# liruiw/OMG-Planner

Measured on AMD Instinct MI355X. Metric: CHOMP iterations/sec (batched scenes) + ms/plan, Panda 7-DoF 30-wp, higher is better.
Workload: dtype f32 SDF / f64 kinematics+update; 1 GPU; 100 table-top scenes/GPU x (64-goal goal-set cost + CHOMP step), Panda 9-dof, 30 waypoints; scenes_per_gpu=100, total_scenes=100, goals=64, waypoints=30, sdf_grid=4x64^3 + 128x96x32 per scene, private, goal_selection=MD on device (omgx_goal_update_optimize), pipeline_parts=3, top_k_collision=1000, plan_restart_every_steps=50

## Files before the change

### include/omg_hip.h

```cpp
#ifndef OMG_HIP_H
#define OMG_HIP_H

#include <stdint.h>

#ifdef __cplusplus
extern "C" {
#endif

#define OMGX_OK 0
#define OMGX_ERR_INVALID (-1)
#define OMGX_ERR_LAUNCH (-2)
#define OMGX_ERR_UNSUPPORTED (-3)

#define OMGX_NUM_LINKS 10
#define OMGX_NUM_DOF 9
#define OMGX_MAX_POINTS 16
#define OMGX_MAX_WAYPOINTS 64
#define OMGX_MAX_CONSTRAINTS 8
#define OMGX_INFO_STRIDE 16

#define OMGX_ROBOT_POSE0 0
#define OMGX_ROBOT_TIP2JOINT 160
#define OMGX_ROBOT_CENTER_OFFSET 320
#define OMGX_ROBOT_JOINT_AXIS 480
// ... 188 lines not shown
                         const int32_t* h_dims, float* out, void* stream);

int32_t omgx_goalset_schedule_len(int32_t num_scenes, int32_t num_goals, int32_t slack);
int omgx_goalset_schedule(const uint32_t* work, const int32_t* active, const int32_t* goal_count, int32_t num_scenes,
                          int32_t num_goals, int32_t slack, int32_t* schedule, void* stream);

int omgx_goalset_schedule_parts(const uint32_t* work, const int32_t* active, const int32_t* goal_count, int32_t num_scenes,
                                int32_t num_goals, int32_t parts, int32_t slack, int32_t* schedule, void* stream);

#define OMGX_SCHEDULE_SCENE_MAJOR 0
#define OMGX_SCHEDULE_LONGEST_FIRST 1
#define OMGX_SCHEDULE_LONGEST_FIRST_MAX_ITEMS 8192
int omgx_goalset_schedule_ordered(const uint32_t* work, const int32_t* active, const int32_t* goal_count, int32_t num_scenes,
                                  int32_t num_goals, int32_t parts, int32_t slack, int32_t order, int32_t* schedule, void* stream);

int64_t omgx_region_scratch_bytes(int32_t dx, int32_t dy, int32_t dz);
int omgx_object_set_grid(omgx_object* object, const float* h_lo, const float* h_hi, const int32_t* h_dims, float delta,
                         int64_t grid_offset, void* stream);
int omgx_fit_influence_region(omgx_object* object, const float* grid, const int32_t* h_dims, const float* h_lo, const float* h_hi,
                              float epsilon, float clearance, void* scratch, void* stream);

int64_t omgx_regions_scratch_bytes(int32_t n_fit, int64_t need_bytes);
int omgx_volume_hashes(const omgx_object* objects, int32_t num_objects, const float* pool, uint64_t* hashes, void* stream);
int omgx_fit_influence_regions(omgx_object* objects, int32_t num_objects, const float* pool, const int32_t* fit_list,
                               const int64_t* need_offsets, int32_t n_fit, int64_t max_voxels, const int32_t* copy_src,
                               void* scratch, void* stream);

typedef struct omgx_plan_iter {
    int32_t mode;
    int32_t start_idx;
// ... 143 lines not shown
```

### omg-planner_amd/csrc/omg_kernels.hip

```cpp
#include <hip/hip_runtime.h>
#include <hip/hip_ext.h>

#include <stdint.h>
#include <stdio.h>
#include <stdlib.h>
#include <string.h>

#include <mutex>

#include "omg_device.h"
#include "omg_host.h"

using namespace omg;

struct RawObjects {
    const float* __restrict__ pose_init;
    const float* __restrict__ sdf_grids;
    const float* __restrict__ sdf_limits;
    const float* __restrict__ eps;
    const float* __restrict__ pad;
    const float* __restrict__ clr;
    const float* __restrict__ dis;
};

#define SDF_LOSS_TILE 32

// ... 671 lines not shown
    if (num_scenes <= 0 || num_goals <= 0 || n_remaining <= 0 || n_points <= 0) return 0;
    (void)n_points;
    return gk_workspace_bytes((int64_t)num_scenes * num_goals, n_remaining);
}

#ifndef GS_LAYER_FOLLOW_MIN
#define GS_LAYER_FOLLOW_MIN 16
#endif
struct GsTiling {
    int goal_parts = 1;
    int layer_lg = 5;
    int layer_cb = 0;
    int spread = 0;
    double* wp_pose_out = nullptr;
    void* kin_ws = nullptr;
};

static inline int gs_parts(int n_remaining, int max_parts) {
    const int ntiles = ((n_remaining + 3) / 4) * 5;
    int np = 1;
    while (np * 2 <= max_parts && ntiles / (np * 2) >= 4) np *= 2;
    return np;
}

static std::atomic<int> g_force_goal_waves{0};
extern "C" void omgx_debug_force_goal_waves(int waves) { g_force_goal_waves.store(waves == 4 || waves == 8 ? waves : 0, std::memory_order_relaxed); }
static inline int gs_wide_waves(int PS, int MR, int P) {
    const int force = g_force_goal_waves.load(std::memory_order_relaxed);
    if (force == 4 || GQ_WAVES != 4 || GqLayout(PS, MR, P, 4, false, 8).total > 64 * 1024) return GQ_WAVES;
    return (force == 8 || GqLayout(PS, MR, P, 4, false, GQ_WAVES).total > 53248) ? 8 : GQ_WAVES;
}
static thread_local int g_last_goalset_variant = 0;
extern "C" int omgx_debug_last_goalset_variant(void) { return g_last_goalset_variant; }

template <class K>
static void gs_launch(K* kernel, unsigned grid, unsigned block, uint32_t lds, hipStream_t st, hipEvent_t ev0, hipEvent_t ev1, const ChunkArgs& ca) {
    if (ev0) hipExtLaunchKernelGGL(kernel, dim3(grid), dim3(block), lds, st, ev0, ev1, 0, ca);
    else hipLaunchKernelGGL(kernel, dim3(grid), dim3(block), lds, st, ca);
}

static int launch_goalset(ChunkArgs& ca, int timing_kind, hipStream_t st, const GsTiling& tl = GsTiling()) {
    const int scene_groups = (ca.S + 7) / 8;
    const bool layer = ca.wp_traj != nullptr;
    if (tl.goal_parts < 1 || tl.goal_parts > 8 || tl.layer_lg < 1 || tl.layer_lg > 10 || 10 % tl.layer_lg != 0 || tl.layer_cb < 0) return OMGX_ERR_INVALID;
    ca.spread = tl.spread != 0;
    ca.NG = ca.NCH;
    ca.NP = ca.NG > 0 ? gs_parts(ca.CH, tl.goal_parts) : 1;
    ca.NCH = ca.NG * ca.NP;
// ... 8 lines not shown
            if (want < ca.wp_n) layer_cb_req = want;
        }
        if (layer && layer_cb_req == 0 && !ca.spread && ca.NG > 0 && tl.layer_lg == 5 && (int64_t)ca.S * ca.NCH <= 1024) {
            ca.layer_lg = 10;
            const int want = ca.CH + 1 > GS_LAYER_FOLLOW_MIN ? ca.CH + 1 : GS_LAYER_FOLLOW_MIN;
            if (want < ca.wp_n) layer_cb_req = want;
        }
    }
    ca.layer_cb = layer ? ((layer_cb_req > 0 && layer_cb_req < ca.wp_n) ? layer_cb_req : ca.wp_n) : 1;
    ca.layer_nb = layer ? (ca.wp_n + ca.layer_cb - 1) / ca.layer_cb : 1;
    ca.layer_parts = ca.layer_lg * ca.layer_nb;
    ca.PS = ca.CH + 1; ca.MR = ca.CH; ca.LPW = 10;
    ca.inv_ncfg = 1.0 / (double)(ca.CH + 1);
    if (layer) { if (ca.layer_cb > ca.PS) ca.PS = ca.layer_cb; if (ca.layer_cb > ca.MR) ca.MR = ca.layer_cb; }
    const int64_t per_scene = (int64_t)ca.NCH + (layer ? ca.layer_parts : 0);
    const int64_t grid = ca.spread ? (int64_t)ca.S * per_scene
                                   : (ca.schedule ? (int64_t)ca.sched_len : (int64_t)scene_groups * ca.NCH * 8) +
                                         (layer ? (int64_t)scene_groups * ca.layer_parts * 8 : 0);
    if (grid > 0x7fffffff) return OMGX_ERR_UNSUPPORTED;
    if (grid == 0) return OMGX_OK;
    const bool pre = tl.kin_ws != nullptr && ca.NG > 0 && ca.traj_start != nullptr;
    const int wide = (!ca.spread && !split && !pre && ca.NG > 0) ? gs_wide_waves(ca.PS, ca.MR, ca.P) : GQ_WAVES;
    ca.tbl_n = gq_choose_tbl_n(ca.PS, ca.MR, ca.P, ca.spread, wide);
    const size_t lds = (size_t)GqLayout(ca.PS, ca.MR, ca.P, ca.tbl_n, ca.spread, wide).total;
    if (lds > 64 * 1024) {
        if (!ca.spread) return OMGX_ERR_UNSUPPORTED;
        int rc = allow_big_lds<10>(k_goalset_queue<2, false, true>, "hipFuncSetAttribute(k_goalset_queue)");
        if (rc != OMGX_OK) return rc;
        rc = allow_big_lds<11>(k_goalset_queue<2, false, true, false, true>, "hipFuncSetAttribute(k_goalset_queue)");
        if (rc != OMGX_OK) return rc;
    }
    ca.pre_poses = nullptr; ca.pre_masks = nullptr;
    if (pre) {
        const int64_t goals = (int64_t)ca.S * ca.NG;
// ... 167 lines not shown

struct GoalsetCall {
    const double* robot = nullptr; int32_t n_points = 0;
    const omgx_object* objects = nullptr; const int32_t* scene_begin = nullptr; const float* sdf_pool = nullptr;
    const double* traj_start = nullptr; int64_t traj_start_stride = 0; const double* goals = nullptr;
    int32_t num_scenes = 0, num_goals = 0, n_remaining = 0, soften_fingers = 0;
    double time_interval = 0.0;
    float *goal_cost = nullptr, *collides = nullptr;
    float* potentials = nullptr;
    void* workspace = nullptr;
    const double* layer_traj = nullptr;
    int32_t layer_n = 0, layer_soften = 0;
    float *layer_pot = nullptr, *layer_grad = nullptr, *layer_col = nullptr;
    const int32_t *active = nullptr, *goal_count = nullptr, *schedule = nullptr;
    int32_t schedule_len = 0; uint32_t* work = nullptr;
    void* stream = nullptr;
    GsTiling tiling;
};

static int goalset_cost_impl(const GoalsetCall& a) {
    if (a.num_scenes < 0 || a.num_goals < 0) return OMGX_ERR_INVALID;
    if (a.num_scenes == 0 || (a.num_goals == 0 && !a.layer_traj)) return OMGX_OK;
    if (!a.robot || !a.objects || !a.scene_begin) return OMGX_ERR_INVALID;
    if (a.num_goals > 0 && (!a.traj_start || !a.goals || !a.goal_cost)) return OMGX_ERR_INVALID;
    if (a.n_points < 1 || a.n_points > OMGX_MAX_POINTS || a.n_remaining < 1 || a.n_remaining > OMGX_MAX_WAYPOINTS)
        return OMGX_ERR_UNSUPPORTED;
    if (!(a.time_interval > 0.0) || (a.num_goals > 0 && a.traj_start_stride < 9)) return OMGX_ERR_INVALID;
    hipStream_t st = (hipStream_t)a.stream;
    const int n = a.num_goals > 0 ? a.n_remaining : 0, C = a.num_goals * n;
    if (a.layer_traj) {
// ... 4 lines not shown
    if ((a.active || a.goal_count || a.schedule || a.work) && a.potentials) return OMGX_ERR_UNSUPPORTED;
    ChunkArgs ca{};
    ca.robot = a.robot; ca.objects = a.objects; ca.scene_begin = a.scene_begin; ca.pool = a.sdf_pool;
    ca.S = a.num_scenes; ca.C = C; ca.CH = n; ca.NCH = a.num_goals; ca.P = a.n_points; ca.soften = a.soften_fingers != 0;
    ca.arc = 1; ca.inv_dt = (float)(1.0 / a.time_interval);
    ca.pot = a.potentials; ca.grad = nullptr; ca.col = nullptr; ca.chunk_cost = a.goal_cost; ca.chunk_col = a.collides;
    ca.traj_start = a.traj_start; ca.ts_stride = a.traj_start_stride; ca.goals = a.goals;
    if (a.layer_traj) {
        ca.wp_traj = a.layer_traj; ca.wp_n = a.layer_n; ca.wp_soften = a.layer_soften != 0;
        ca.wp_pot = a.layer_pot; ca.wp_grad = a.layer_grad; ca.wp_col = a.layer_col;
    }
    if (a.schedule && (a.schedule_len < 8 || a.schedule_len % 8 != 0)) return OMGX_ERR_INVALID;
    ca.active = a.active; ca.goal_count = a.goal_count; ca.schedule = a.schedule; ca.sched_len = a.schedule ? a.schedule_len : 0; ca.work = a.work;
    GsTiling tl = a.tiling;
    tl.kin_ws = a.workspace;
    return a.potentials ? launch_chunks(ca, st) : launch_goalset(ca, 0, st, tl);
}

extern "C" int omgx_goalset_cost(const double* robot, int32_t n_points, const omgx_object* objects,
                                 const int32_t* scene_begin, const float* sdf_pool, const double* traj_start,
                                 int64_t traj_start_stride, const double* goals, int32_t num_scenes, int32_t num_goals,
                                 int32_t n_remaining,
                                 double time_interval, int32_t soften_fingers, float* goal_cost, float* potentials,
                                 float* collides, void* workspace, const int32_t* active, const int32_t* goal_count, void* stream) {
    GoalsetCall a;
    a.robot = robot; a.n_points = n_points; a.objects = objects; a.scene_begin = scene_begin; a.sdf_pool = sdf_pool;
    a.traj_start = traj_start; a.traj_start_stride = traj_start_stride; a.goals = goals; a.num_scenes = num_scenes; a.num_goals = num_goals;
    a.n_remaining = n_remaining; a.time_interval = time_interval; a.soften_fingers = soften_fingers;
    a.goal_cost = goal_cost; a.potentials = potentials; a.collides = collides; a.workspace = workspace;
    a.active = active; a.goal_count = goal_count; a.stream = stream;
    return goalset_cost_impl(a);
}

#define SCH_TPB 1024
#define SCH_LDS_ITEMS 14336
struct SchedArgs {
    const uint32_t* work;
    const int32_t* active;
    const int32_t* goal_count;
    int S, G, slack, slots, staged;
    int32_t* sched;
    int np;
    int longest_first;
};

__global__ __launch_bounds__(SCH_TPB) void k_goalset_schedule(SchedArgs a) {
    extern __shared__ unsigned long long sch_lds[];
    const int S = a.S, G = a.G, tid = threadIdx.x;
    unsigned long long* Ws = sch_lds;
    unsigned long long* Wc = Ws + S;
    unsigned long long* offw = Wc + S;
    uint32_t* nval = reinterpret_cast<uint32_t*>(offw + S);
    uint32_t* offp = nval + S;
    uint32_t* srank = offp + S;
    uint32_t* wl = srank + S;
    unsigned char* xs = reinterpret_cast<unsigned char*>(wl + S * G);
    __shared__ unsigned long long tot[2];
    __shared__ uint32_t cnt_all;
    __shared__ uint32_t first[8];
    __shared__ uint32_t first_r[8];
    __shared__ uint32_t cnt_r[8];
    auto item_w = [&](int s, int g) -> uint32_t {
        if (a.staged) return wl[s * G + g];
        if ((a.active && a.active[s] == 0) || (a.goal_count && g / a.np >= a.goal_count[s])) return 0u;
        const uint32_t w = a.work ? a.work[(size_t)s * G + g] : 1u;
        return w ? w : 1u;
    };
    if (tid == 0) { tot[0] = tot[1] = 0ull; cnt_all = 0u; }
    if (tid < 8) { first[tid] = 0xffffffffu; first_r[tid] = 0xffffffffu; cnt_r[tid] = 0u; }
    for (int i = tid; i < a.slots * 8; i += SCH_TPB) a.sched[i] = -1;
    if (a.staged)
        for (int i = tid; i < S * G; i += SCH_TPB) {
            const int s = i / G, g = i - s * G;
            uint32_t w = 0u;
            if (!((a.active && a.active[s] == 0) || (a.goal_count && g / a.np >= a.goal_count[s]))) {
                w = a.work ? a.work[i] : 1u;
                w = w ? w : 1u;
            }
            wl[i] = w;
        }
    __syncthreads();
    for (int s = tid; s < S; s += SCH_TPB) {
        unsigned long long w = 0;
        uint32_t n = 0;
// ... 53 lines not shown
        pos = offp[s] + r;
        const unsigned long long c2 = 2ull * (offw[s] + before) + wclamp(w);
        const unsigned long long xx = (8ull * c2) / (2ull * total_c);
        x = xx > 7 ? 7 : (int)xx;
        const unsigned long long r2 = 2ull * (offr[s] + before_r) + w;
        const unsigned long long xq = (8ull * r2) / (2ull * total_r);
        xr = xq > 7 ? 7 : (int)xq;
    };
    uint32_t kpos[4];
    int kx[4], kxr[4];
    int kept_n = 0;
    for (int i = tid; i < S * G; i += SCH_TPB) {
        const int s = i / G, g = i - s * G;
        const uint32_t w = item_w(s, g);
        uint32_t pos = 0; int x = -1, xr = -1;
        if (w) { place(s, g, w, pos, x, xr); atomicMin(&first[x], pos); atomicMin(&first_r[xr], pos); atomicAdd(&cnt_r[xr], 1u); }
        if (kept_n < 4) { kpos[kept_n] = pos; kx[kept_n] = x; kxr[kept_n] = xr; }
        ++kept_n;
        if (a.longest_first) xs[i] = (unsigned char)(w ? (x | (xr << 4)) : 255);
    }
    __syncthreads();
    bool use_raw = true;
#pragma unroll
    for (int x = 0; x < 8; ++x) use_raw = use_raw && cnt_r[x] <= (uint32_t)a.slots;
    if (a.longest_first) {
        for (int i = tid; i < S * G; i += SCH_TPB) {
            const uint32_t w = wl[i];
            if (!w) continue;
            const int sh = use_raw ? 4 : 0;
            const unsigned char x = (xs[i] >> sh) & 7;
            uint32_t r = 0;
#pragma unroll 4
            for (int j = 0; j < S * G; ++j) r += (wl[j] != 0u && ((xs[j] >> sh) & 7) == x && (wl[j] > w || (wl[j] == w && j < i))) ? 1u : 0u;
            if ((int)r < a.slots) a.sched[(size_t)r * 8 + x] = i;
        }
        return;
    }
    int k = 0;
    for (int i = tid; i < S * G; i += SCH_TPB, ++k) {
// ... 32 lines not shown
    if (parts != 1 && parts != 2 && parts != 4 && parts != 8) return OMGX_ERR_INVALID;
    if (order != OMGX_SCHEDULE_SCENE_MAJOR && order != OMGX_SCHEDULE_LONGEST_FIRST) return OMGX_ERR_INVALID;
    return goalset_schedule_impl(work, active, goal_count, num_scenes, num_goals, parts, slack, schedule, stream, order);
}

static int goalset_schedule_impl(const uint32_t* work, const int32_t* active, const int32_t* goal_count, int32_t num_scenes,
                                 int32_t num_goals_, int32_t parts, int32_t slack, int32_t* schedule, void* stream, int32_t order) {
    if (num_scenes <= 0 || num_goals_ <= 0 || slack < 1 || !schedule) return OMGX_ERR_INVALID;
    const int64_t items64 = (int64_t)num_goals_ * parts;
    if (items64 > 65536) return OMGX_ERR_UNSUPPORTED;
    const int32_t num_goals = (int32_t)items64;
    if ((int64_t)num_scenes * num_goals > 65536 || num_scenes > OMGX_SCHEDULE_MAX_SCENES) return OMGX_ERR_UNSUPPORTED;
    const int items = num_scenes * num_goals;
    const int staged = (items <= SCH_LDS_ITEMS && num_scenes <= 128) ? 1 : 0;
    const int longest_first = (order == OMGX_SCHEDULE_LONGEST_FIRST && staged && items <= OMGX_SCHEDULE_LONGEST_FIRST_MAX_ITEMS) ? 1 : 0;
    SchedArgs a{work, active, goal_count, num_scenes, num_goals, slack, omgx_goalset_schedule_len(num_scenes, num_goals, slack) / 8, staged, schedule, parts, longest_first};
    const size_t lds = (size_t)num_scenes * (3 * sizeof(unsigned long long) + 3 * sizeof(uint32_t)) + (staged ? (size_t)items * sizeof(uint32_t) : 0) +
                       (longest_first ? (size_t)items : 0);
    hipLaunchKernelGGL(k_goalset_schedule, dim3(1), dim3(SCH_TPB), lds, (hipStream_t)stream, a);
    OMGX_CHECK_LAUNCH("k_goalset_schedule");
    return OMGX_OK;
}

extern "C" int omgx_goalset_cost_layer(const double* robot, int32_t n_points, const omgx_object* objects,
                                       const int32_t* scene_begin, const float* sdf_pool, const double* traj_start,
                                       int64_t traj_start_stride, const double* goals, int32_t num_scenes, int32_t num_goals,
                                       int32_t n_remaining, double time_interval, int32_t soften_fingers, float* goal_cost,
                                       float* collides, void* workspace, const double* traj, int32_t n_waypoints,
                                       int32_t layer_soften_fingers, float* layer_potentials, float* layer_grads,
                                       float* layer_collides, const int32_t* active, const int32_t* goal_count,
                                       const int32_t* schedule, int32_t schedule_len, uint32_t* work, void* stream) {
    if (!traj) return OMGX_ERR_INVALID;
    GoalsetCall a;
    a.robot = robot; a.n_points = n_points; a.objects = objects; a.scene_begin = scene_begin; a.sdf_pool = sdf_pool;
    a.traj_start = traj_start; a.traj_start_stride = traj_start_stride; a.goals = goals; a.num_scenes = num_scenes; a.num_goals = num_goals;
    a.n_remaining = n_remaining; a.time_interval = time_interval; a.soften_fingers = soften_fingers;
    a.goal_cost = goal_cost; a.collides = collides; a.workspace = workspace;
    a.layer_traj = traj; a.layer_n = n_waypoints; a.layer_soften = layer_soften_fingers; a.layer_pot = layer_potentials; a.layer_grad = layer_grads; a.layer_col = layer_collides;
    a.active = active; a.goal_count = goal_count; a.schedule = schedule; a.schedule_len = schedule_len; a.work = work; a.stream = stream;
    return goalset_cost_impl(a);
}

extern "C" int omgx_goalset_cost_layer_parts(const double* robot, int32_t n_points, const omgx_object* objects,
                                             const int32_t* scene_begin, const float* sdf_pool, const double* traj_start,
                                             int64_t traj_start_stride, const double* goals, int32_t num_scenes, int32_t num_goals,
                                             int32_t n_remaining, double time_interval, int32_t soften_fingers, float* goal_cost,
                                             float* collides, const double* traj, int32_t n_waypoints,
                                             int32_t layer_soften_fingers, float* layer_potentials, float* layer_grads,
                                             float* layer_collides, const int32_t* active, const int32_t* goal_count,
                                             const int32_t* schedule, int32_t schedule_len, uint32_t* work, int32_t goal_parts,
                                             double* layer_poses, void* workspace, void* stream) {
    if (!traj) return OMGX_ERR_INVALID;
    GoalsetCall a;
    a.robot = robot; a.n_points = n_points; a.objects = objects; a.scene_begin = scene_begin; a.sdf_pool = sdf_pool;
    a.traj_start = traj_start; a.traj_start_stride = traj_start_stride; a.goals = goals; a.num_scenes = num_scenes; a.num_goals = num_goals;
    a.n_remaining = n_remaining; a.time_interval = time_interval; a.soften_fingers = soften_fingers;
    a.goal_cost = goal_cost; a.collides = collides; a.workspace = workspace;
    a.layer_traj = traj; a.layer_n = n_waypoints; a.layer_soften = layer_soften_fingers; a.layer_pot = layer_potentials; a.layer_grad = layer_grads; a.layer_col = layer_collides;
    a.active = active; a.goal_count = goal_count; a.schedule = schedule; a.schedule_len = schedule_len; a.work = work; a.stream = stream;
    a.tiling.goal_parts = goal_parts; a.tiling.wp_pose_out = layer_poses;
    return goalset_cost_impl(a);
}

extern "C" int32_t omgx_goalset_parts(int32_t n_remaining, int32_t goal_parts) {
    if (n_remaining < 1 || goal_parts < 1 || goal_parts > 8) return 0;
    return gs_parts(n_remaining, goal_parts);
}

extern "C" int omgx_goalset_cost_layer_tiled(const double* robot, int32_t n_points, const omgx_object* objects,
                                             const int32_t* scene_begin, const float* sdf_pool, const double* traj_start,
                                             int64_t traj_start_stride, const double* goals, int32_t num_scenes, int32_t num_goals,
                                             int32_t n_remaining, double time_interval, int32_t soften_fingers, float* goal_cost,
                                             float* collides, const double* traj, int32_t n_waypoints, int32_t layer_soften_fingers,
                                             float* layer_potentials, float* layer_grads, float* layer_collides,
                                             const int32_t* active, const int32_t* goal_count, int32_t goal_parts,
                                             int32_t layer_link_groups, int32_t layer_config_block, int32_t spread, double* layer_poses,
// ... 146 lines not shown
```

### omg-planner_amd/engine.py

```python
from __future__ import annotations

import operator

import numpy as np
import torch

from . import _lib, ops
from .config import Config
from .robot import PandaModel
from .scenes import SceneBatch


def shard_range(num_items: int, rank: int, world: int) -> range:
    base, rem = divmod(num_items, world)
    lo = rank * base + min(rank, rem)
    return range(lo, lo + base + (1 if rank < rem else 0))


_SIDE_STREAMS: dict = {}


def _side_stream(device: torch.device, i: int) -> "torch.cuda.Stream":
    key = (device.index if device.index is not None else torch.cuda.current_device(), i)
    st = _SIDE_STREAMS.get(key)
# ... 150 lines not shown
        self.learner_state = ops.learner_state(S, G, dev, goal_counts)
        self.cost_vec = dzeros((S, G), np.float64)
        self.eta = float(np.sqrt(np.log(G + 1) / cfg.optim_steps))
        self._active = torch.from_numpy(np.ones(S, np.int32)).to(dev)
        self._masked = False
        self.step_count = 0
        self.t = 0
        self._scene_flags = dzeros(S, np.int32)
        self.work = dzeros(S * G * (1 if self.latency else self._parts_max), np.int32)
        self.auto_schedule = True
        self.schedule = None
        self._sched_np = 1
        self._gs_launches = 0
        self._measured = False
        self._sched_buf, self._sched_flip, self._sched_age = None, 0, None
        self._uniform_cache = None
        self._ticket_src = [0]
        self._measure_fence = [None]
        with torch.cuda.device(dev):
            self._num_cus = int(_lib.lib().omgx_device_cu_count())
        if self._num_cus <= 0:
            self._num_cus = torch.cuda.get_device_properties(dev).multi_processor_count
        self._parts, self._forked, self._in_plan = None, False, False
        self._hot = None
        self._capturing = False
        self._scratch_state = self._cubic_h = self._cubic_tmp = self._cubic_diff = None

    @property
    def active(self) -> torch.Tensor:
        return self._active
# ... 105 lines not shown
            tot += parts[:, :, j]
        return tot

    def _make_part(self, lo: int, hi: int, stream):
        import copy
        part = object.__new__(ChompEngine)
        part.__dict__.update(self.__dict__)
        part.cfg = copy.copy(self.cfg)
        part.S, part.stream, part._lo = hi - lo, stream, lo
        part._batch_scenes = self.S
        part._parts, part._forked, part.pipeline = None, False, 1
        part._hot = None
        part.scenes = self.scenes.scene_range(lo, hi)
        part.work = torch.zeros(part.S * self.G * (1 if self.latency else self._parts_max), dtype=torch.int32, device=self.device)
        part.schedule, part._gs_launches, part._measured, part._sched_np = None, 0, False, 1
        part._sched_buf, part._sched_flip, part._sched_age = None, 0, None
        part._uniform_cache = None
        if self.goal_count is not None:
            part._goal_counts_host = self._goal_counts_host[lo:hi]
        self._bind_part(part)
        return part

    def _bind_part(self, part):
        lo, hi = part._lo, part._lo + part.S
        for k in self._PART_TENSORS:
            v = getattr(self, k)
            setattr(part, k, None if v is None else v[lo:hi])

    def _refresh_parts(self):
        for part in self._parts or ():
            self._bind_part(part)
# ... 108 lines not shown
                else:
                    self.schedule = self.build_schedule(active=self._mask(), parts=NP, uniform=rebuild == "masked-uniform")
        return (self.schedule if use else None), (self.work[:items] if measure else None)

    def _dispatch_measured(self, NP: int):
        self._measured = True
        with torch.cuda.stream(self.stream):
            self.schedule = self.build_schedule(parts=NP)

    def _goalset_layer(self, prm: _lib.LearnerParams, calls: "ops.IterationCalls", stream: int):
        self._gs_launches += 1
        NP = self._parts_last = max(1, int(prm.cost_parts))
        schedule, work = (None, None) if self.latency else self._dispatch(NP)
        calls.use_layer_poses = self._poses_on
        if work is None:
            calls.goalset_layer(prm.start_idx, self._masked, schedule, None, stream)
            return
        mine = self.stream if self.stream is not None else torch.cuda.current_stream(self.device)
        fence = self._measure_fence
        if fence[0] is not None:
            mine.wait_event(fence[0])
        calls.goalset_layer(prm.start_idx, self._masked, schedule, work, stream)
        fence[0] = mine.record_event()
        self._dispatch_measured(NP)

    def _uniform_schedule(self, parts: int = 1) -> torch.Tensor:
        S, G = self.S, self.G * parts
        if self.goal_count is not None:
            items = np.concatenate([s * G + np.arange(int(c) * parts) for s, c in enumerate(self._goal_counts_host)])
        else:
            items = np.arange(S * G)
        n = len(items)
        pos = np.arange(n)
        x = np.minimum(8 * pos // max(n, 1), 7)
        first = np.searchsorted(x, np.arange(8))
        rank = pos - first[x]
        slots = int(rank.max()) + 1 if n else 1
        sched = np.full(slots * 8, -1, np.int32)
        sched[rank * 8 + x] = items
        return torch.as_tensor(sched, device=self.device)

    def build_schedule(self, active: "torch.Tensor | None" = None, uniform: bool = False, parts: int = 1) -> torch.Tensor:
        self._sched_np = parts
        if self.S * self.G * parts > 65536 or self.S > _lib.SCHEDULE_MAX_SCENES:
            if self._uniform_cache is None:
                self._uniform_cache = {}
            if parts not in self._uniform_cache:
                self._uniform_cache[parts] = self._uniform_schedule(parts)
            return self._uniform_cache[parts]
        if self._sched_buf is None:
            self._sched_buf = {}
        self._sched_flip ^= 1
        key = (parts, self._sched_flip)
        out = ops.goalset_schedule(None if uniform else self.work[: self.S * self.G * parts], self.S, self.G, active=active, goal_count=self.goal_count,
                                   slack=self.schedule_slack, out=self._sched_buf.get(key), device=self.device, parts=parts,
                                   longest_first=(not uniform) and self.S * self.G * parts <= self.LONGEST_FIRST_MAX_ITEMS)
        self._sched_buf[key] = out
        return out

    def _layer(self):
        if self.latency:
            ops.goalset_cost_layer_tiled(self.robot, self.P, self.scenes, None, None, 1, self.cfg.time_interval, self.traj,
                                         (self.pot, self.pgrad, self.col), None, layer_soften_fingers=self.cfg.uncheck_finger_collision == -1,
                                         layer_link_groups=self.LAT_LAYER_LINK_GROUPS,
                                         layer_config_block=self.LAT_LAYER_BLOCK, spread=True,
                                         layer_poses=self.wp_pose if self._poses_on else None)
            return
        if self._poses_on:
            ops.goalset_cost_layer_tiled(self.robot, self.P, self.scenes, None, None, 1, self.cfg.time_interval, self.traj,
                                         (self.pot, self.pgrad, self.col), None, layer_soften_fingers=self.cfg.uncheck_finger_collision == -1,
                                         goal_parts=1, layer_link_groups=5, layer_config_block=0, spread=False, layer_poses=self.wp_pose)
            return
# ... 263 lines not shown

    def _plan_all_done(self, early_stop: bool, t: int) -> bool:
        if self._capturing:
            return False
        if not (early_stop and self.S <= 4 and t in _ALL_DONE_CHECKS):
            return False
        self.join()
        return not self._active.cpu().numpy().any()

    def capture_plan(self, early_stop: bool = True, initial_goal: bool = True) -> "PlanGraph":
        state = self.snapshot()
        self.plan(early_stop, initial_goal)
        self.restore(state)
        torch.cuda.synchronize(self.device)
        graph = torch.cuda.CUDAGraph()
        self._capturing = True
        try:
            with torch.cuda.graph(graph):
                info = self.plan(early_stop, initial_goal)
                self.join()
        finally:
            self._capturing = False
        self.restore(state)
        torch.cuda.synchronize(self.device)
        return PlanGraph(self, graph, info)

    def final_costs(self) -> torch.Tensor:
        self.join()
        return self.info[:, 0].contiguous()

# ... 47 lines not shown
```

### omg-planner_amd/ops.py

```python
from __future__ import annotations

import ctypes as C
import time
from collections import Counter

import numpy as np
import torch

from . import _lib, scenes as _sc
from ._lib import ChompParams, LearnerParams, check

_ws_cache: dict = {}


def _ptr(t):
    return None if t is None else C.c_void_p(t.data_ptr())


def _stream():
    return C.c_void_p(torch.cuda.current_stream().cuda_stream)


def _need(t: torch.Tensor, dtype, name: str):
    if not t.is_cuda:
# ... 462 lines not shown
        cost, col = out
    pots = torch.empty((S, G, n_remaining, 10, P), dtype=torch.float32, device=dev) if want_potentials else None
    cost_p, col_p = _goal_out((cost, col), S * G)
    l = _lib.lib()
    with torch.cuda.device(dev):
        ws = _kin_workspace(prepass, S, G, n_remaining, P, dev) if not want_potentials else None
        check(l.omgx_goalset_cost(_ptr(robot), P, _ptr(scenes.objects), _ptr(scenes.scene_begin), _ptr(scenes.pool),
                                  ts, ts_stride, _ptr(goals), S, G, n_remaining, float(dt), int(bool(soften_fingers)),
                                  cost_p, _ptr(pots), col_p, _ptr(ws), _ptr(_active(active, S)), _ptr(_active(goal_count, S)),
                                  _stream()), "omgx_goalset_cost")
    return cost, col, pots


def goalset_cost_layer(robot, P, scenes: DeviceScenes, traj_start, goals, n_remaining, dt, traj, layer_out, soften_fingers=False,
                       layer_soften_fingers=False, out=None, active=None, goal_count=None, schedule=None, work=None, goal_parts=1,
                       layer_poses=None, prepass=False):
    start = _traj_start(traj_start)
    _need(goals, torch.float64, "goals")
    S, G = goals.shape[0], goals.shape[1]
    layer = _layer(S, P, traj, layer_out, layer_poses)
    dev = goals.device
    NP = goalset_parts(n_remaining, goal_parts) if int(goal_parts) != 1 else 1
    if NP < 1:
        raise _lib.OmgHipError("goal_parts must be 1, 2, 4 or 8")
    if out is None:
        cost = torch.empty((S, G) if NP == 1 else (S, G, NP), dtype=torch.float32, device=dev)
        col = torch.empty((S, G) if NP == 1 else (S, G, NP), dtype=torch.float32, device=dev)
    else:
        cost, col = out
    l = _lib.lib()
    with torch.cuda.device(dev):
        g = _GoalsetArgs(robot, P, scenes, goals, S, G, dt, soften_fingers, _goal_out((cost, col), S * G * NP), layer, layer_soften_fingers,
                         _active(goal_count, S), _kin_workspace(prepass, S, G, n_remaining, P, dev))
        active = _ptr(_active(active, S))
        if int(goal_parts) != 1 or layer_poses is not None:
            check(l.omgx_goalset_cost_layer_parts(*g.parts(start, n_remaining, active, schedule, work, NP, int(goal_parts), g.poses, _stream())),
                  "omgx_goalset_cost_layer_parts")
        else:
            check(l.omgx_goalset_cost_layer(*g.whole(start, n_remaining, active, schedule, work, _stream())), "omgx_goalset_cost_layer")
    return cost, col


def goalset_parts(n_remaining: int, goal_parts: int) -> int:
    return int(_lib.lib().omgx_goalset_parts(int(n_remaining), int(goal_parts)))


def goalset_cost_layer_tiled(robot, P, scenes: DeviceScenes, traj_start, goals, n_remaining, dt, traj, layer_out, out,
                             soften_fingers=False, layer_soften_fingers=False, active=None, goal_count=None, goal_parts=4,
                             layer_link_groups=10, layer_config_block=16, spread=True, layer_poses=None, prepass=False):
# ... 35 lines not shown
        out = torch.empty(n, dtype=torch.int32, device=device)
    _i32n(out, n, "schedule")
    _i32n(work, num_scenes * num_goals * parts, "work")
    with torch.cuda.device(out.device):
        if longest_first:
            check(l.omgx_goalset_schedule_ordered(_ptr(work), _ptr(_active(active, num_scenes)), _ptr(_active(goal_count, num_scenes)),
                                                  num_scenes, num_goals, parts, slack, _lib.SCHEDULE_LONGEST_FIRST, _ptr(out), _stream()),
                  "omgx_goalset_schedule_ordered")
        elif parts != 1:
            check(l.omgx_goalset_schedule_parts(_ptr(work), _ptr(_active(active, num_scenes)), _ptr(_active(goal_count, num_scenes)),
                                                num_scenes, num_goals, parts, slack, _ptr(out), _stream()), "omgx_goalset_schedule_parts")
        else:
            check(l.omgx_goalset_schedule(_ptr(work), _ptr(_active(active, num_scenes)), _ptr(_active(goal_count, num_scenes)), num_scenes,
                                          num_goals, slack, _ptr(out), _stream()), "omgx_goalset_schedule")
    return out


def forward_kinematics(robot, P, joints, want_joint_info=True):
    _need(joints, torch.float64, "joints")
    B, dev = joints.shape[0], joints.device
    poses = torch.empty((B, 10, 4, 4), dtype=torch.float64, device=dev)
    org = torch.empty((B, 10, 3), dtype=torch.float64, device=dev) if want_joint_info else None
    ax = torch.empty((B, 10, 3), dtype=torch.float64, device=dev) if want_joint_info else None
    with torch.cuda.device(dev):
        check(_lib.lib().omgx_forward_kinematics(_ptr(robot), P, _ptr(joints), B, _ptr(poses), _ptr(org), _ptr(ax), _stream()),
              "omgx_forward_kinematics")
    return poses, org, ax


def pose_table(robot, P, configs: torch.Tensor, out: "torch.Tensor | None" = None) -> torch.Tensor:
# ... 165 lines not shown
        n = layer[1]
        self._tiling = None if tiling is None else tuple(int(v) for v in tiling)
        self._goal_parts = int(goal_parts) if self._tiling is None else 1
        max_parts = self._tiling[0] if self._tiling is not None else self._goal_parts
        goal_ptrs = _goal_out(goal_out, S * G * (goalset_parts(n, max_parts) if max_parts != 1 else 1))
        _iteration_tensors(S, goal_set, reach, state, goal_idx, cost_vector, start, end, goal_rows, goal_point, step_out, active, goal_count,
                           eta, scene_flags)
        self.S, self.G, self.n, self.P, self.dt = S, G, n, int(P), float(dt)
        self.device = traj.device
        self._dev_index = traj.device.index if traj.device.index is not None else torch.cuda.current_device()
        self._traj_addr = traj.data_ptr()
        l = _lib.lib()
        self._f_gs, self._f_up = l.omgx_goalset_cost_layer, l.omgx_goal_update_optimize
        self._f_gst = l.omgx_goalset_cost_layer_tiled
        self._f_gsp = l.omgx_goalset_cost_layer_parts
        self.kin_workspace = (torch.empty(max(16, l.omgx_goalset_workspace_bytes(S, G, n, self.P)), dtype=torch.uint8, device=traj.device)
                              if prepass else None)
        self._gs = _GoalsetArgs(robot, P, scenes, goals, S, G, dt, False, goal_ptrs, layer, layer_soften_fingers, goal_count, self.kin_workspace)
        self._layer_alone = _GoalsetArgs(robot, P, scenes, None, S, 0, dt, False, (None, None), layer, layer_soften_fingers, None, None)
        p = _ptr
        self._active_p = p(active)
        traj_p, _n, lp, lg, lc, _poses = layer
        grad, cost_traj, info = step_out
        self._up_a = (p(goal_set), p(reach), goal_ptrs[0], p(state), p(goal_idx), p(cost_vector), p(robot))
        self._up_b = (traj_p, p(start), p(end), p(goal_rows), p(goal_point), lp, lg, lc, p(active), S, p(grad), p(cost_traj), p(info), None)
        self._flags, self._eta = p(scene_flags), p(eta)
        self.use_layer_poses = False

    def goalset_layer(self, start_idx: int, masked: bool, schedule, work, stream):
        g, start, n_remaining = self._gs, (C.c_void_p(self._traj_addr + 72 * start_idx), self.n * 9), self.n - start_idx
        active, poses, stream = self._active_p if masked else None, g.poses if self.use_layer_poses else None, C.c_void_p(stream)
        if self._tiling is not None:
            if schedule is not None or work is not None:
                raise _lib.OmgHipError("a tiled goal-set launch takes no dispatch schedule")
            self._call(self._f_gst, g.tiled(start, n_remaining, active, self._tiling, poses, stream))
        elif self._goal_parts > 1 or self.use_layer_poses:
            NP = goalset_parts(n_remaining, self._goal_parts) if self._goal_parts > 1 else 1
            self._call(self._f_gsp, g.parts(start, n_remaining, active, schedule, work, NP, self._goal_parts, poses, stream))
        else:
            self._call(self._f_gs, g.whole(start, n_remaining, active, schedule, work, stream))

    def _call(self, fn, args):
        if torch.cuda.current_device() == self._dev_index:
            check(fn(*args), fn.__name__)
        else:
            with torch.cuda.device(self.device):
                check(fn(*args), fn.__name__)

    LAYER_ONLY_TILING = None

    def _layer_only_tiling(self):
        if self.LAYER_ONLY_TILING is not None:
            return self.LAYER_ONLY_TILING
        S = getattr(self, "batch_scenes", self.S)
# ... 648 lines not shown
```

Before: 559,300 iterations/s.

## Shrink goal-set launch grid to occupied schedule rows via mapped host word

The schedule kernel now counts occupied rows per column and publishes the maximum, tagged with a generation, into a mapped pinned host word. When the goal-set launch gets a matching token, the host reads that word and sizes the grid to rows*8 instead of the full slack-padded schedule length. This avoids launching workgroups that would find only empty (-1) slots and exit. In exchange the host must observe the device-written value, which presumes the schedule kernel has already finished. It falls back to the full grid when the generation does not match, and tokens are disabled during graph capture.

```diff
diff --git a/include/omg_hip.h b/include/omg_hip.h
--- a/include/omg_hip.h
+++ b/include/omg_hip.h
@@ -226,6 +226,9 @@
 int omgx_goalset_schedule_ordered(const uint32_t* work, const int32_t* active, const int32_t* goal_count, int32_t num_scenes,
                                   int32_t num_goals, int32_t parts, int32_t slack, int32_t order, int32_t* schedule, void* stream);
 
+int64_t omgx_goalset_schedule_token(const int32_t* schedule);
+int omgx_goalset_schedule_use_token(int64_t token);
+
 int64_t omgx_region_scratch_bytes(int32_t dx, int32_t dy, int32_t dz);
 int omgx_object_set_grid(omgx_object* object, const float* h_lo, const float* h_hi, const int32_t* h_dims, float delta,
                          int64_t grid_offset, void* stream);
diff --git a/omg-planner_amd/csrc/omg_kernels.hip b/omg-planner_amd/csrc/omg_kernels.hip
--- a/omg-planner_amd/csrc/omg_kernels.hip
+++ b/omg-planner_amd/csrc/omg_kernels.hip
@@ -10,6 +10,7 @@
 
 #include "omg_device.h"
 #include "omg_host.h"
+#include "omg_sched_rows.h"
 
 using namespace omg;
 
@@ -711,6 +712,7 @@
     int spread = 0;
     double* wp_pose_out = nullptr;
     void* kin_ws = nullptr;
+    int64_t sched_token = 0;
 };
 
 static inline int gs_parts(int n_remaining, int max_parts) {
@@ -729,6 +731,29 @@
 }
 static thread_local int g_last_goalset_variant = 0;
 extern "C" int omgx_debug_last_goalset_variant(void) { return g_last_goalset_variant; }
+static thread_local int g_last_goalset_grid = 0;
+extern "C" int omgx_debug_last_goalset_grid(void) { return g_last_goalset_grid; }
+
+static omg_sched::Registry g_sched_rows;
+static std::once_flag g_sched_rows_once;
+static void sched_rows_attach() {
+    std::call_once(g_sched_rows_once, [] {
+        void* h = nullptr;
+        void* d = nullptr;
+        const size_t bytes = sizeof(uint64_t) * omg_sched::SLOTS;
+        if (hipHostMalloc(&h, bytes, hipHostMallocMapped | hipHostMallocPortable) != hipSuccess || !h) { (void)hipGetLastError(); return; }
+        memset(h, 0, bytes);
+        if (hipHostGetDevicePointer(&d, h, 0) != hipSuccess || d != h) { (void)hipGetLastError(); (void)hipHostFree(h); return; }
+        g_sched_rows.attach(static_cast<uint64_t*>(h));
+    });
+}
+static bool sched_rows_capturing(hipStream_t st) {
+    hipStreamCaptureStatus cs = hipStreamCaptureStatusNone;
+    if (hipStreamIsCapturing(st, &cs) != hipSuccess) { (void)hipGetLastError(); return true; }
+    return cs != hipStreamCaptureStatusNone;
+}
+static thread_local int64_t g_next_sched_token = 0;
+static int64_t take_sched_token() { const int64_t t = g_next_sched_token; g_next_sched_token = 0; return t; }
 
 template <class K>
 static void gs_launch(K* kernel, unsigned grid, unsigned block, uint32_t lds, hipStream_t st, hipEvent_t ev0, hipEvent_t ev1, const ChunkArgs& ca) {
@@ -767,10 +792,14 @@
     ca.inv_ncfg = 1.0 / (double)(ca.CH + 1);
     if (layer) { if (ca.layer_cb > ca.PS) ca.PS = ca.layer_cb; if (ca.layer_cb > ca.MR) ca.MR = ca.layer_cb; }
     const int64_t per_scene = (int64_t)ca.NCH + (layer ? ca.layer_parts : 0);
-    const int64_t grid = ca.spread ? (int64_t)ca.S * per_scene
-                                   : (ca.schedule ? (int64_t)ca.sched_len : (int64_t)scene_groups * ca.NCH * 8) +
-                                         (layer ? (int64_t)scene_groups * ca.layer_parts * 8 : 0);
+    int64_t goal_wgs = ca.schedule ? (int64_t)ca.sched_len : (int64_t)scene_groups * ca.NCH * 8;
+    if (ca.schedule && tl.sched_token != 0 && !ca.spread) {
+        const int64_t rows = g_sched_rows.rows(tl.sched_token, ca.schedule);
+        if (rows >= 0 && rows * 8 <= goal_wgs && !sched_rows_capturing(st)) goal_wgs = rows * 8;
+    }
+    const int64_t grid = ca.spread ? (int64_t)ca.S * per_scene : goal_wgs + (layer ? (int64_t)scene_groups * ca.layer_parts * 8 : 0);
     if (grid > 0x7fffffff) return OMGX_ERR_UNSUPPORTED;
+    g_last_goalset_grid = (int)grid;
     if (grid == 0) return OMGX_OK;
     const bool pre = tl.kin_ws != nullptr && ca.NG > 0 && ca.traj_start != nullptr;
     const int wide = (!ca.spread && !split && !pre && ca.NG > 0) ? gs_wide_waves(ca.PS, ca.MR, ca.P) : GQ_WAVES;
@@ -968,6 +997,7 @@
     float *layer_pot = nullptr, *layer_grad = nullptr, *layer_col = nullptr;
     const int32_t *active = nullptr, *goal_count = nullptr, *schedule = nullptr;
     int32_t schedule_len = 0; uint32_t* work = nullptr;
+    int64_t sched_token = 0;
     void* stream = nullptr;
     GsTiling tiling;
 };
@@ -1002,6 +1032,7 @@
     ca.active = a.active; ca.goal_count = a.goal_count; ca.schedule = a.schedule; ca.sched_len = a.schedule ? a.schedule_len : 0; ca.work = a.work;
     GsTiling tl = a.tiling;
     tl.kin_ws = a.workspace;
+    tl.sched_token = a.sched_token;
     return a.potentials ? launch_chunks(ca, st) : launch_goalset(ca, 0, st, tl);
 }
 
@@ -1030,6 +1061,8 @@
     int32_t* sched;
     int np;
     int longest_first;
+    unsigned long long* rows_word;
+    uint32_t rows_gen;
 };
 
 __global__ __launch_bounds__(SCH_TPB) void k_goalset_schedule(SchedArgs a) {
@@ -1048,6 +1081,7 @@
     __shared__ uint32_t first[8];
     __shared__ uint32_t first_r[8];
     __shared__ uint32_t cnt_r[8];
+    __shared__ uint32_t cnt_c[8];
     auto item_w = [&](int s, int g) -> uint32_t {
         if (a.staged) return wl[s * G + g];
         if ((a.active && a.active[s] == 0) || (a.goal_count && g / a.np >= a.goal_count[s])) return 0u;
@@ -1055,7 +1089,7 @@
         return w ? w : 1u;
     };
     if (tid == 0) { tot[0] = tot[1] = 0ull; cnt_all = 0u; }
-    if (tid < 8) { first[tid] = 0xffffffffu; first_r[tid] = 0xffffffffu; cnt_r[tid] = 0u; }
+    if (tid < 8) { first[tid] = 0xffffffffu; first_r[tid] = 0xffffffffu; cnt_r[tid] = 0u; cnt_c[tid] = 0u; }
     for (int i = tid; i < a.slots * 8; i += SCH_TPB) a.sched[i] = -1;
     if (a.staged)
         for (int i = tid; i < S * G; i += SCH_TPB) {
@@ -1139,7 +1173,7 @@
         const int s = i / G, g = i - s * G;
         const uint32_t w = item_w(s, g);
         uint32_t pos = 0; int x = -1, xr = -1;
-        if (w) { place(s, g, w, pos, x, xr); atomicMin(&first[x], pos); atomicMin(&first_r[xr], pos); atomicAdd(&cnt_r[xr], 1u); }
+        if (w) { place(s, g, w, pos, x, xr); atomicMin(&first[x], pos); atomicMin(&first_r[xr], pos); atomicAdd(&cnt_r[xr], 1u); atomicAdd(&cnt_c[x], 1u); }
         if (kept_n < 4) { kpos[kept_n] = pos; kx[kept_n] = x; kxr[kept_n] = xr; }
         ++kept_n;
         if (a.longest_first) xs[i] = (unsigned char)(w ? (x | (xr << 4)) : 255);
@@ -1148,6 +1182,13 @@
     bool use_raw = true;
 #pragma unroll
     for (int x = 0; x < 8; ++x) use_raw = use_raw && cnt_r[x] <= (uint32_t)a.slots;
+    if (a.rows_word && tid == 0) {
+        uint32_t rows = 0u;
+#pragma unroll
+        for (int x = 0; x < 8; ++x) { const uint32_t c = use_raw ? cnt_r[x] : cnt_c[x]; rows = c > rows ? c : rows; }
+        if (rows > (uint32_t)a.slots) rows = (uint32_t)a.slots;
+        __hip_atomic_store(a.rows_word, ((unsigned long long)a.rows_gen << 32) | rows, __ATOMIC_RELAXED, __HIP_MEMORY_SCOPE_SYSTEM);
+    }
     if (a.longest_first) {
         for (int i = tid; i < S * G; i += SCH_TPB) {
             const uint32_t w = wl[i];
@@ -1210,7 +1251,14 @@
     const int items = num_scenes * num_goals;
     const int staged = (items <= SCH_LDS_ITEMS && num_scenes <= 128) ? 1 : 0;
     const int longest_first = (order == OMGX_SCHEDULE_LONGEST_FIRST && staged && items <= OMGX_SCHEDULE_LONGEST_FIRST_MAX_ITEMS) ? 1 : 0;
-    SchedArgs a{work, active, goal_count, num_scenes, num_goals, slack, omgx_goalset_schedule_len(num_scenes, num_goals, slack) / 8, staged, schedule, parts, longest_first};
+    SchedArgs a{work, active, goal_count, num_scenes, num_goals, slack, omgx_goalset_schedule_len(num_scenes, num_goals, slack) / 8, staged, schedule, parts, longest_first,
+                nullptr, 0u};
+    {
+        const bool live = !sched_rows_capturing((hipStream_t)stream);
+        if (live) sched_rows_attach();
+        uint64_t* word = nullptr;
+        if (g_sched_rows.begin_build(schedule, live, &word, &a.rows_gen)) a.rows_word = reinterpret_cast<unsigned long long*>(word);
+    }
     const size_t lds = (size_t)num_scenes * (3 * sizeof(unsigned long long) + 3 * sizeof(uint32_t)) + (staged ? (size_t)items * sizeof(uint32_t) : 0) +
                        (longest_first ? (size_t)items : 0);
     hipLaunchKernelGGL(k_goalset_schedule, dim3(1), dim3(SCH_TPB), lds, (hipStream_t)stream, a);
@@ -1226,8 +1274,10 @@
                                        int32_t layer_soften_fingers, float* layer_potentials, float* layer_grads,
                                        float* layer_collides, const int32_t* active, const int32_t* goal_count,
                                        const int32_t* schedule, int32_t schedule_len, uint32_t* work, void* stream) {
+    const int64_t token = take_sched_token();
     if (!traj) return OMGX_ERR_INVALID;
     GoalsetCall a;
+    a.sched_token = token;
     a.robot = robot; a.n_points = n_points; a.objects = objects; a.scene_begin = scene_begin; a.sdf_pool = sdf_pool;
     a.traj_start = traj_start; a.traj_start_stride = traj_start_stride; a.goals = goals; a.num_scenes = num_scenes; a.num_goals = num_goals;
     a.n_remaining = n_remaining; a.time_interval = time_interval; a.soften_fingers = soften_fingers;
@@ -1246,8 +1296,10 @@
                                              float* layer_collides, const int32_t* active, const int32_t* goal_count,
                                              const int32_t* schedule, int32_t schedule_len, uint32_t* work, int32_t goal_parts,
                                              double* layer_poses, void* workspace, void* stream) {
+    const int64_t token = take_sched_token();
     if (!traj) return OMGX_ERR_INVALID;
     GoalsetCall a;
+    a.sched_token = token;
     a.robot = robot; a.n_points = n_points; a.objects = objects; a.scene_begin = scene_begin; a.sdf_pool = sdf_pool;
     a.traj_start = traj_start; a.traj_start_stride = traj_start_stride; a.goals = goals; a.num_scenes = num_scenes; a.num_goals = num_goals;
     a.n_remaining = n_remaining; a.time_interval = time_interval; a.soften_fingers = soften_fingers;
@@ -1256,6 +1308,14 @@
     a.active = active; a.goal_count = goal_count; a.schedule = schedule; a.schedule_len = schedule_len; a.work = work; a.stream = stream;
     a.tiling.goal_parts = goal_parts; a.tiling.wp_pose_out = layer_poses;
     return goalset_cost_impl(a);
+}
+
+extern "C" int64_t omgx_goalset_schedule_token(const int32_t* schedule) { return g_sched_rows.token(schedule); }
+
+extern "C" int omgx_goalset_schedule_use_token(int64_t token) {
+    if (token < 0) return OMGX_ERR_INVALID;
+    g_next_sched_token = token;
+    return OMGX_OK;
 }
 
 extern "C" int32_t omgx_goalset_parts(int32_t n_remaining, int32_t goal_parts) {
diff --git a/omg-planner_amd/csrc/omg_sched_rows.h b/omg-planner_amd/csrc/omg_sched_rows.h
--- /dev/null
+++ b/omg-planner_amd/csrc/omg_sched_rows.h
@@ -0,0 +1,92 @@
+#ifndef OMG_SCHED_ROWS_H
+#define OMG_SCHED_ROWS_H
+
+#include <stdint.h>
+
+#include <mutex>
+
+namespace omg_sched {
+
+constexpr int SLOTS = 64;
+
+inline uint64_t pack_word(uint32_t generation, uint32_t rows) { return ((uint64_t)generation << 32) | rows; }
+
+class Registry {
+   public:
+    void attach(uint64_t* words) {
+        std::lock_guard<std::mutex> g(mu_);
+        if (!words_) words_ = words;
+    }
+    bool attached() {
+        std::lock_guard<std::mutex> g(mu_);
+        return words_ != nullptr;
+    }
+    bool begin_build(const void* buf, bool publish, uint64_t** word, uint32_t* generation) {
+        std::lock_guard<std::mutex> g(mu_);
+        if (!words_ || !buf) return false;
+        int at = find(buf);
+        if (at < 0) {
+            if (!publish) return false;
+            at = oldest();
+            slots_[at].buf = buf;
+        }
+        Slot& s = slots_[at];
+        s.generation = s.generation + 1u ? s.generation + 1u : 1u;
+        s.built = ++clock_;
+        s.published = publish;
+        if (!publish) return false;
+        *word = words_ + at;
+        *generation = s.generation;
+        return true;
+    }
+    void set_generation(const void* buf, uint32_t generation) {
+        std::lock_guard<std::mutex> g(mu_);
+        const int at = find(buf);
+        if (at >= 0) slots_[at].generation = generation;
+    }
+    int64_t token(const void* buf) {
+        std::lock_guard<std::mutex> g(mu_);
+        const int at = buf ? find(buf) : -1;
+        if (at < 0 || !slots_[at].published || slots_[at].generation == 0u) return 0;
+        return (int64_t)(((uint64_t)(at + 1) << 32) | slots_[at].generation);
+    }
+    int64_t rows(int64_t token, const void* buf) {
+        if (token <= 0 || !buf) return -1;
+        const uint64_t t = (uint64_t)token;
+        const uint32_t generation = (uint32_t)t;
+        const uint64_t at1 = t >> 32;
+        if (at1 < 1 || at1 > (uint64_t)SLOTS || generation == 0u) return -1;
+        std::lock_guard<std::mutex> g(mu_);
+        const Slot& s = slots_[at1 - 1];
+        if (!words_ || s.buf != buf || !s.published || s.generation != generation) return -1;
+        const uint64_t w = __atomic_load_n(words_ + (at1 - 1), __ATOMIC_ACQUIRE);
+        if ((uint32_t)(w >> 32) != generation) return -1;
+        return (int64_t)(uint32_t)w;
+    }
+
+   private:
+    struct Slot {
+        const void* buf = nullptr;
+        uint32_t generation = 0;
+        uint64_t built = 0;
+        bool published = false;
+    };
+    int find(const void* buf) const {
+        for (int i = 0; i < SLOTS; ++i)
+            if (slots_[i].buf == buf) return i;
+        return -1;
+    }
+    int oldest() const {
+        int at = 0;
+        for (int i = 1; i < SLOTS; ++i)
+            if (slots_[i].built < slots_[at].built) at = i;
+        return at;
+    }
+    std::mutex mu_;
+    Slot slots_[SLOTS];
+    uint64_t clock_ = 0;
+    uint64_t* words_ = nullptr;
+};
+
+}
+#endif
diff --git a/omg-planner_amd/engine.py b/omg-planner_amd/engine.py
--- a/omg-planner_amd/engine.py
+++ b/omg-planner_amd/engine.py
@@ -188,6 +188,8 @@
         self._gs_launches = 0
         self._measured = False
         self._sched_buf, self._sched_flip, self._sched_age = None, 0, None
+        self._sched_token = 0
+        self._sched_tokens_on = [True]
         self._uniform_cache = None
         self._ticket_src = [0]
         self._measure_fence = [None]
@@ -323,7 +325,7 @@
         part.scenes = self.scenes.scene_range(lo, hi)
         part.work = torch.zeros(part.S * self.G * (1 if self.latency else self._parts_max), dtype=torch.int32, device=self.device)
         part.schedule, part._gs_launches, part._measured, part._sched_np = None, 0, False, 1
-        part._sched_buf, part._sched_flip, part._sched_age = None, 0, None
+        part._sched_buf, part._sched_flip, part._sched_age, part._sched_token = None, 0, None, 0
         part._uniform_cache = None
         if self.goal_count is not None:
             part._goal_counts_host = self._goal_counts_host[lo:hi]
@@ -462,13 +464,13 @@
         schedule, work = (None, None) if self.latency else self._dispatch(NP)
         calls.use_layer_poses = self._poses_on
         if work is None:
-            calls.goalset_layer(prm.start_idx, self._masked, schedule, None, stream)
+            calls.goalset_layer(prm.start_idx, self._masked, schedule, None, stream, self._sched_token)
             return
         mine = self.stream if self.stream is not None else torch.cuda.current_stream(self.device)
         fence = self._measure_fence
         if fence[0] is not None:
             mine.wait_event(fence[0])
-        calls.goalset_layer(prm.start_idx, self._masked, schedule, work, stream)
+        calls.goalset_layer(prm.start_idx, self._masked, schedule, work, stream, self._sched_token)
         fence[0] = mine.record_event()
         self._dispatch_measured(NP)
 
@@ -490,6 +492,7 @@
 
     def build_schedule(self, active: "torch.Tensor | None" = None, uniform: bool = False, parts: int = 1) -> torch.Tensor:
         self._sched_np = parts
+        self._sched_token = 0
         if self.S * self.G * parts > 65536 or self.S > _lib.SCHEDULE_MAX_SCENES:
             if self._uniform_cache is None:
                 self._uniform_cache = {}
@@ -504,6 +507,7 @@
                                    slack=self.schedule_slack, out=self._sched_buf.get(key), device=self.device, parts=parts,
                                    longest_first=(not uniform) and self.S * self.G * parts <= self.LONGEST_FIRST_MAX_ITEMS)
         self._sched_buf[key] = out
+        self._sched_token = ops.goalset_schedule_token(out) if self._sched_tokens_on[0] else 0
         return out
 
     def _layer(self):
@@ -797,6 +801,9 @@
         self.restore(state)
         torch.cuda.synchronize(self.device)
         graph = torch.cuda.CUDAGraph()
+        self._sched_tokens_on[0] = False
+        for e in [self] + list(self._parts or []):
+            e._sched_token = 0
         self._capturing = True
         try:
             with torch.cuda.graph(graph):
diff --git a/omg-planner_amd/ops.py b/omg-planner_amd/ops.py
--- a/omg-planner_amd/ops.py
+++ b/omg-planner_amd/ops.py
@@ -500,7 +500,7 @@
 
 def goalset_cost_layer(robot, P, scenes: DeviceScenes, traj_start, goals, n_remaining, dt, traj, layer_out, soften_fingers=False,
                        layer_soften_fingers=False, out=None, active=None, goal_count=None, schedule=None, work=None, goal_parts=1,
-                       layer_poses=None, prepass=False):
+                       layer_poses=None, prepass=False, schedule_token=0):
     start = _traj_start(traj_start)
     _need(goals, torch.float64, "goals")
     S, G = goals.shape[0], goals.shape[1]
@@ -519,6 +519,8 @@
         g = _GoalsetArgs(robot, P, scenes, goals, S, G, dt, soften_fingers, _goal_out((cost, col), S * G * NP), layer, layer_soften_fingers,
                          _active(goal_count, S), _kin_workspace(prepass, S, G, n_remaining, P, dev))
         active = _ptr(_active(active, S))
+        if schedule is not None and schedule_token:
+            check(l.omgx_goalset_schedule_use_token(int(schedule_token)), "omgx_goalset_schedule_use_token")
         if int(goal_parts) != 1 or layer_poses is not None:
             check(l.omgx_goalset_cost_layer_parts(*g.parts(start, n_remaining, active, schedule, work, NP, int(goal_parts), g.poses, _stream())),
                   "omgx_goalset_cost_layer_parts")
@@ -584,6 +586,10 @@
             check(l.omgx_goalset_schedule(_ptr(work), _ptr(_active(active, num_scenes)), _ptr(_active(goal_count, num_scenes)), num_scenes,
                                           num_goals, slack, _ptr(out), _stream()), "omgx_goalset_schedule")
     return out
+
+
+def goalset_schedule_token(schedule) -> int:
+    return int(_lib.lib().omgx_goalset_schedule_token(_ptr(schedule)))
 
 
 def forward_kinematics(robot, P, joints, want_joint_info=True):
@@ -779,6 +785,7 @@
         self._f_gs, self._f_up = l.omgx_goalset_cost_layer, l.omgx_goal_update_optimize
         self._f_gst = l.omgx_goalset_cost_layer_tiled
         self._f_gsp = l.omgx_goalset_cost_layer_parts
+        self._f_tok = l.omgx_goalset_schedule_use_token
         self.kin_workspace = (torch.empty(max(16, l.omgx_goalset_workspace_bytes(S, G, n, self.P)), dtype=torch.uint8, device=traj.device)
                               if prepass else None)
         self._gs = _GoalsetArgs(robot, P, scenes, goals, S, G, dt, False, goal_ptrs, layer, layer_soften_fingers, goal_count, self.kin_workspace)
@@ -792,7 +799,7 @@
         self._flags, self._eta = p(scene_flags), p(eta)
         self.use_layer_poses = False
 
-    def goalset_layer(self, start_idx: int, masked: bool, schedule, work, stream):
+    def goalset_layer(self, start_idx: int, masked: bool, schedule, work, stream, schedule_token: int = 0):
         g, start, n_remaining = self._gs, (C.c_void_p(self._traj_addr + 72 * start_idx), self.n * 9), self.n - start_idx
         active, poses, stream = self._active_p if masked else None, g.poses if self.use_layer_poses else None, C.c_void_p(stream)
         if self._tiling is not None:
@@ -800,9 +807,13 @@
                 raise _lib.OmgHipError("a tiled goal-set launch takes no dispatch schedule")
             self._call(self._f_gst, g.tiled(start, n_remaining, active, self._tiling, poses, stream))
         elif self._goal_parts > 1 or self.use_layer_poses:
+            if schedule is not None and schedule_token:
+                self._f_tok(schedule_token)
             NP = goalset_parts(n_remaining, self._goal_parts) if self._goal_parts > 1 else 1
             self._call(self._f_gsp, g.parts(start, n_remaining, active, schedule, work, NP, self._goal_parts, poses, stream))
         else:
+            if schedule is not None and schedule_token:
+                self._f_tok(schedule_token)
             self._call(self._f_gs, g.whole(start, n_remaining, active, schedule, work, stream))
 
     def _call(self, fn, args):
```

Result: no change. 562,600 iterations/s, median of 2 (+0.6%).
